# wnmusic/simpleFE

Measured on AMD Instinct MI355X. Metric: complex-float32 MS/s through 256-tap blkconv FIR; % of HBM roofline, higher is better.
Workload: dtype f32

## Files before the change

simplefe_amd/csrc/poly_gen.hip:

```cpp
#include <stdint.h>

#include <type_traits>

#ifdef SFE_DIAG
#include <stdlib.h>
#endif

#include "common.h"
#include "fft16.h"

namespace sfe {
namespace {

struct RunLds {
    double t0;
    float d;
    int k0;
    int count, pad;
};
static_assert(sizeof(RunLds) == 24, "TlSeg layout");

constexpr int GEN_MAX_RUNS = 1024;

template <int KPT, bool REAL, bool IN_U8, bool NOPRO = false>
__global__ __launch_bounds__(256, KPT <= 9 ? 3 : 2) void poly_gen4096_kernel(PolyGenArgs a)
{
    constexpr int NC = REAL ? 3 : 2;
    typedef typename std::conditional<REAL, float, v2f>::type E;
    __shared__ v2f lds[FFT_ROWS * LDS_K2_STRIDE];
    __shared__ unsigned tab_pos[KPT * 256];
    __shared__ float tab_mu[KPT * 256];
    __shared__ int s_bound[2 * NC], s_run[NC];
    const unsigned t = threadIdx.x, lo = t & 15u, hi = t >> 4;
    const int ch = blockIdx.y;
    const long long blk = (REAL ? 2 : 1) * (long long)blockIdx.x;
    const E *in = static_cast<const E *>(a.in) + (size_t)ch * a.in_stride;
    const E *hist = static_cast<const E *>(a.hist) + (size_t)ch * a.hl;
    E *out = static_cast<E *>(a.out) + (size_t)ch * a.out_stride;
    const int A = a.adv, U = a.U;

    v2f nx[16];
    const long long base = blk * A - a.ovl;
    if constexpr (IN_U8) {
        const unsigned char *in8 = static_cast<const unsigned char *>(a.in) + (size_t)ch * a.in_stride * (REAL ? 1 : 2);
        auto at = [&](long long i) -> E {
            if (i >= 0) {
                if (i >= a.n_in) return E{};
                if constexpr (REAL) return u8_to_f32(in8[i]);
                else return (v2f){u8_to_f32(in8[2 * i]), u8_to_f32(in8[2 * i + 1])};
            }
            return i >= -(long long)a.hl ? hist[a.hl + i] : E{};
        };
#pragma unroll
        for (int r = 0; r < 16; r++) {
            const long long i = base + 256 * r + (long long)t;
            if constexpr (REAL) nx[r] = (v2f){at(i), at(i + A)};
            else nx[r] = at(i);
        }
    } else if constexpr (!REAL) {
        if (base >= 0 && base + FFT_N <= a.n_in) {
#pragma unroll
            for (int r = 0; r < 16; r++) nx[r] = __builtin_nontemporal_load(in + base + 256 * r + t);
        } else {
#pragma unroll
            for (int r = 0; r < 16; r++) {
                const long long i = base + 256 * r + (long long)t;
                if (i >= 0) nx[r] = i < a.n_in ? in[i] : (v2f){0.0f, 0.0f};
                else nx[r] = i >= -(long long)a.hl ? hist[a.hl + i] : (v2f){0.0f, 0.0f};
            }
        }
    } else {
        if (base >= 0 && base + A + FFT_N <= a.n_in) {
#pragma unroll
            for (int r = 0; r < 16; r++)
                nx[r] = (v2f){__builtin_nontemporal_load(in + base + 256 * r + t), __builtin_nontemporal_load(in + base + A + 256 * r + t)};
        } else {
            auto at = [&](long long i) -> float {
                if (i >= 0) return i < a.n_in ? in[i] : 0.0f;
                return i >= -(long long)a.hl ? hist[a.hl + i] : 0.0f;
            };
#pragma unroll
            for (int r = 0; r < 16; r++) {
                const long long i = base + 256 * r + (long long)t;
                nx[r] = (v2f){at(i), at(i + A)};
            }
        }
    }

    int T = 0;
    long long k_first = 0;
    if constexpr (NOPRO) {
        T = a.diag_T < 256 * KPT ? a.diag_T : 256 * KPT;
        k_first = (long long)blockIdx.x * T;
        const unsigned Uu = (unsigned)U, e0 = (unsigned)a.ovl - 1u;
#pragma unroll
        for (int q = 0; q < KPT; q++) {
            const unsigned idx = t + 256u * q;
            const unsigned pl = (unsigned)(((unsigned long long)idx * (unsigned)A * Uu) / (unsigned)(T > 0 ? T : 1));
            const unsigned n = pl / Uu, ph = pl - n * Uu, e = e0 + (n < (unsigned)A ? n : (unsigned)A - 1u);
            const bool wrap = ph + 1u == Uu;
            const unsigned cell = (e >> 8) * LDS_K2_STRIDE + (e & 255u);
            const unsigned dcell = wrap ? ((e & 255u) == 255u ? LDS_K2_STRIDE - 255u : 1u) : 0u;
            tab_pos[idx] = (int)idx < T ? ((cell << 19) | (dcell << 10) | ((wrap ? 0u : ph + 1u) << 5) | ph) : (31u | (31u << 5));
            tab_mu[idx] = 0.25f;
        }
    } else {
    const long long Plo = (long long)U * (blk * A - 1), Phi = Plo + (long long)(REAL ? 2 : 1) * U * A;
    const long long BU = (long long)a.blksize * U;
    auto fdiv = [&](long long x) -> long long {
        if (x < 0) return 0;
        long long c = (long long)((double)x / (double)BU);
        if (c * BU > x) c--;
        if ((c + 1) * BU <= x) c++;
        return c;
    };
    long long c_first = fdiv(Plo + 1), c_last = fdiv(Phi);
    if (c_last >= a.n_chunks) c_last = a.n_chunks - 1;
    if (c_first > c_last) c_first = c_last;
    if (c_last > c_first + NC - 1) c_last = c_first + NC - 1;
    const int ncalls = (int)(c_last - c_first) + 1;
    SegChunk cc[NC];
    int nsg[NC], rbase[NC + 1];
    rbase[0] = 0;
#pragma unroll
    for (int i = 0; i < NC; i++) {
        cc[i] = a.chunks[c_first + (i < ncalls ? i : 0)];
        nsg[i] = i < ncalls ? cc[i].n_seg : 0;
        rbase[i + 1] = rbase[i] + nsg[i];
    }
    RunLds *runs = reinterpret_cast<RunLds *>(lds);
    {
        unsigned long long *ws = reinterpret_cast<unsigned long long *>(lds);
#pragma unroll
        for (int i = 0; i < NC; i++) {
            const unsigned long long *g = reinterpret_cast<const unsigned long long *>(static_cast<const RunLds *>(a.segs) + cc[i].seg_first);
            for (int j = (int)t; j < 3 * nsg[i]; j += 256) ws[3 * rbase[i] + j] = g[j];
        }
    }
    lds_barrier();
    auto count_below = [&](const RunLds *rs, int n_seg, int n_out, long long bound, int *run) -> int {
        *run = 0;
        if (n_seg == 0 || bound <= -1) return 0;
        const double bd = (double)bound;
        int l = 0, h = n_seg;
        while (l < h) {
            const int m = (l + h) >> 1;
            if (rs[m].t0 < bd) l = m + 1; else h = m;
        }
        if (l == 0) return 0;
        const RunLds g = rs[l - 1];
        long long i = g.count;
        if (g.count > 1 && g.d > 0.0f) {
            i = (long long)ceil((bd - g.t0) / (double)g.d);
            if (i < 0) i = 0;
            if (i > g.count) i = g.count;
            while (i < g.count && g.t0 + (double)i * (double)g.d < bd) i++;
            while (i > 0 && g.t0 + (double)(i - 1) * (double)g.d >= bd) i--;
        }
        *run = i < g.count ? l - 1 : l;
        const int k = g.k0 + (int)i;
        return k < n_out ? k : n_out;
    };
    const unsigned w = __builtin_amdgcn_readfirstlane(t >> 6), lane = t & 63u;
#pragma unroll
    for (int sx = 0; sx < 2 * NC; sx += 4) {
        const int sb = sx + (int)w;
        if (sb < 2 * NC) {
            int run = 0, r = 0;
#pragma unroll
            for (int i = 0; i < NC; i++)
                if (i == (sb >> 1) && i < ncalls)
                    r = count_below(runs + rbase[i], nsg[i], cc[i].n_out, ((sb & 1) ? Phi : Plo) - cc[i].in_off * U, &run);
            if (lane == 0) {
                s_bound[sb] = r;
                if (!(sb & 1)) s_run[sb >> 1] = run;
            }
        }
    }
    lds_barrier();
    int k_lo[NC], n_part[NC], idx_base[NC + 1], run_lo[NC];
    idx_base[0] = 0;
    k_first = cc[0].k_first + __builtin_amdgcn_readfirstlane(s_bound[0]);
    bool have_first = false;
#pragma unroll
    for (int i = 0; i < NC; i++) {
        k_lo[i] = __builtin_amdgcn_readfirstlane(s_bound[2 * i]);
        n_part[i] = __builtin_amdgcn_readfirstlane(s_bound[2 * i + 1]) - k_lo[i];
        run_lo[i] = __builtin_amdgcn_readfirstlane(s_run[i]);
        idx_base[i + 1] = idx_base[i] + n_part[i];
        if (!have_first && n_part[i] > 0) {
            k_first = cc[i].k_first + k_lo[i];
            have_first = true;
        }
    }
    T = idx_base[NC];
    if (T == 0) return;

#pragma unroll
    for (int q = 0; q < KPT; q++)
        if ((int)t + 256 * q >= T) {
            tab_pos[256 * q + t] = 31u | (31u << 5);
            tab_mu[256 * q + t] = 0.0f;
        }
    const unsigned Uu = (unsigned)U, Minv = Uu > 1u ? 0xFFFFFFFFu / Uu + 1u : 0u;
    const unsigned e0 = (unsigned)a.ovl - 1u;
#pragma unroll
    for (int part = 0; part < NC; part++) {
        const RunLds *rs = runs + rbase[part];
        const int ns = nsg[part];
        const unsigned off32 = (unsigned)(cc[part].in_off * U - Plo);
        int lu = run_lo[part];
        if (lu > ns - 1) lu = ns - 1;
#pragma unroll 1
        for (int c = (int)w; 64 * c < n_part[part]; c += 4) {
            const int kk0 = k_lo[part] + 64 * c;
            while (lu + 1 < ns && __builtin_amdgcn_readfirstlane(rs[lu].k0 + rs[lu].count) <= kk0) lu++;
            const int i_part = 64 * c + (int)lane;
            if (i_part < n_part[part]) {
                const int kk = kk0 + (int)lane;
                int l = lu;
                while (rs[l].k0 + rs[l].count <= kk) l++;
                const RunLds g = rs[l];
                const double tt = g.t0 + (double)(kk - g.k0) * (double)g.d;
                const double fl = floor(tt);
                const float mu = (float)(tt - fl);
                const unsigned pl = off32 + (unsigned)(int)fl;
                unsigned n = Uu > 1u ? __umulhi(pl, Minv) : pl;
                const unsigned ph = pl - n * Uu;
                unsigned half = 0u;
                if (REAL && n >= (unsigned)A) {
                    n -= (unsigned)A;
                    half = 1u;
                }
                const unsigned e = e0 + n;
                const bool wrap = ph + 1u == Uu;
                const unsigned cell = (e >> 8) * LDS_K2_STRIDE + (e & 255u);
                const unsigned dcell = wrap ? ((e & 255u) == 255u ? LDS_K2_STRIDE - 255u : 1u) : 0u;
                tab_pos[idx_base[part] + i_part] = (cell << 19) | (half << 15) | (dcell << 10) | ((wrap ? 0u : ph + 1u) << 5) | ph;
                tab_mu[idx_base[part] + i_part] = mu;
            }
        }
    }
    }
    lds_barrier();

    v2f p1[4], q1[4], p2[4], q2[4];
    auto load_tw1 = [&]() {
        unsigned tt = t;
        asm volatile("" : "+v"(tt));
#pragma unroll
        for (int k = 1; k < 4; k++) {
            p1[k] = a.tw1[k * 256 + tt];
            q1[k] = a.tw1[(k + 3) * 256 + tt];
        }
    };
    auto load_tw2 = [&]() {
        unsigned ll = lo;
        asm volatile("" : "+v"(ll));
#pragma unroll
        for (int k = 1; k < 4; k++) {
            p2[k] = a.tw2[k * 16 + ll];
            q2[k] = a.tw2[(k + 3) * 16 + ll];
        }
    };
    load_tw1();
    load_tw2();
    const unsigned base_b = hi * LDS_K2_STRIDE + lo, base_c = hi * LDS_K2_STRIDE + lo * LDS_K1_STRIDE;

    dft16<-1>(nx);
#pragma unroll
    for (int k = 0; k < 16; k++) {
        v2f x = nx[P16(k)];
        if ((k >> 2) && (k & 3)) x = cmul2(x, q1[k >> 2], p1[k & 3]);
        else if (k >> 2) x = cmul(x, q1[k >> 2]);
        else if (k & 3) x = cmul(x, p1[k & 3]);
        lds[t + (unsigned)k * LDS_K2_STRIDE] = x;
    }
    lds_barrier();
    v2f v[16];
#pragma unroll
    for (int r = 0; r < 16; r++) v[r] = lds[base_b + 16u * r];
    dft16<-1>(v);
    lds_barrier();
#pragma unroll
    for (int k = 0; k < 16; k++) {
        v2f x = v[P16(k)];
        if ((k >> 2) && (k & 3)) x = cmul2(x, q2[k >> 2], p2[k & 3]);
        else if (k >> 2) x = cmul(x, q2[k >> 2]);
        else if (k & 3) x = cmul(x, p2[k & 3]);
        lds[base_b + (unsigned)LDS_K1_STRIDE * k] = x;
    }
    lds_barrier();
    v2f hn[16];
    auto load_h = [&](int j) {
        unsigned tt = t;
        asm volatile("" : "+v"(tt));
        const v2f *hs = a.hs + (size_t)j * 16 * 256;
#pragma unroll
        for (int k = 0; k < 16; k++) hn[k] = hs[k * 256 + tt];
    };
    load_h(0);
    v2f X[16];
#pragma unroll
    for (int r = 0; r < 16; r++) X[r] = lds[base_c + r];
    dft16<-1>(X);

    E acc[KPT];
#pragma unroll
    for (int q = 0; q < KPT; q++) acc[q] = E{};
#pragma unroll 1
    for (int j = 0; j < U; j++) {
        lds_barrier();
#pragma unroll
        for (int k = 0; k < 16; k++) v[P16(k)] = cmul(X[P16(k)], hn[k]);
        if (j + 1 < U) load_h(j + 1);
        load_tw1();
        dft16_rev<+1>(v);
#pragma unroll
        for (int k = 0; k < 16; k++) lds[base_c + k] = v[k];
        lds_barrier();
#pragma unroll
        for (int r = 0; r < 16; r++) {
            v2f x = lds[base_b + (unsigned)LDS_K1_STRIDE * r];
            if ((r >> 2) && (r & 3)) x = cmul2_conj(x, q2[r >> 2], p2[r & 3]);
            else if (r >> 2) x = cmul_conj(x, q2[r >> 2]);
            else if (r & 3) x = cmul_conj(x, p2[r & 3]);
            v[r] = x;
        }
        dft16<+1>(v);
        lds_barrier();
#pragma unroll
        for (int k = 0; k < 16; k++) lds[base_b + 16u * k] = v[P16(k)];
        lds_barrier();
#pragma unroll
        for (int r = 0; r < 16; r++) {
            v2f x = lds[t + (unsigned)r * LDS_K2_STRIDE];
            if ((r >> 2) && (r & 3)) x = cmul2_conj(x, q1[r >> 2], p1[r & 3]);
            else if (r >> 2) x = cmul_conj(x, q1[r >> 2]);
            else if (r & 3) x = cmul_conj(x, p1[r & 3]);
            v[r] = x;
        }
        dft16<+1>(v);
#pragma unroll
        for (int r = 0; r < 16; r++) lds[t + (unsigned)r * LDS_K2_STRIDE] = v[P16(r)];
        lds_barrier();
        const unsigned ju = (unsigned)j;
        const char *lb = reinterpret_cast<const char *>(lds);
#pragma unroll
        for (int q = 0; q < KPT; q++) {
            const unsigned pw = tab_pos[256 * q + t];
            const float mu_q = tab_mu[256 * q + t];
            const float w0 = (pw & 31u) == ju ? 1.0f - mu_q : 0.0f;
            const float w1 = ((pw >> 5) & 31u) == ju ? mu_q : 0.0f;
            if constexpr (!REAL) {
                const unsigned a0 = pw >> 16;
                const v2f s0 = *reinterpret_cast<const v2f *>(lb + a0);
                const v2f s1 = *reinterpret_cast<const v2f *>(lb + a0 + (((pw >> 10) & 31u) << 3));
                acc[q] = __builtin_elementwise_fma((v2f){w0, w0}, s0, acc[q]);
                acc[q] = __builtin_elementwise_fma((v2f){w1, w1}, s1, acc[q]);
            } else {
                const unsigned a0 = (pw >> 16) + ((pw >> 13) & 4u);
                const float s0 = *reinterpret_cast<const float *>(lb + a0);
                const float s1 = *reinterpret_cast<const float *>(lb + a0 + (((pw >> 10) & 31u) << 3));
                acc[q] = __builtin_fmaf(w0, s0, acc[q]);
                acc[q] = __builtin_fmaf(w1, s1, acc[q]);
            }
        }
    }
#pragma unroll
    for (int q = 0; q < KPT; q++)
        if ((int)t + 256 * q < T) __builtin_nontemporal_store(acc[q], out + k_first + (long long)t + 256 * q);
}

}

int poly_gen_outputs_per_block(int U, int adv, float step)
{
    const double span = (double)U * adv;
    return (int)(span / ((double)step * (1.0 - 1.0 / 4194304.0))) + 2;
}

int launch_poly_gen(const PolyGenArgs &a0, int max_runs, float step, int n_channels, hipStream_t s)
{
    if (a0.n_chunks <= 0) return SFE_OK;
    PolyGenArgs a = a0;
    if (a.ovl < a.plen || a.ovl >= FFT_N / 2 || (a.ovl & 15) || max_runs > GEN_MAX_RUNS) return SFE_ESTATE;
    if (a.U > 31 || (long long)a.blksize * a.U >= 0x7fffffffLL) return SFE_ESTATE;
    const int per_wg = a.real ? 2 : 1, kpt_max = a.real ? 22 : 16;
    a.adv = FFT_N - a.ovl;
    if (poly_gen_outputs_per_block(a.U, per_wg * a.adv, step) > 256 * kpt_max) {
        a.adv = (int)((256.0 * kpt_max - 2) * (double)step * (1.0 - 1.0 / 4194304.0) / (a.U * per_wg)) & ~15;
        if (a.adv < 512 || poly_gen_outputs_per_block(a.U, per_wg * a.adv, step) > 256 * kpt_max) return SFE_ESTATE;
    }
    if (a.blksize < a.adv) return SFE_ESTATE;
    const int per_block = poly_gen_outputs_per_block(a.U, per_wg * a.adv, step);
    const long long A = a.adv;
    const long long nblk = (a.n_in / A + 1 + per_wg - 1) / per_wg;
    if (nblk > 0x7fffffffLL) return SFE_ESTATE;
    dim3 grid((unsigned)nblk, (unsigned)n_channels), block(256);
    const int kpt = (per_block + 255) / 256;
#ifdef SFE_DIAG
    if (const char *e = getenv("SFE_GEN_NOPRO"))
        if (atoi(e) && !a.real && !a.in_u8 && kpt <= 9) {
            a.diag_T = per_block - 3;
            hipLaunchKernelGGL((poly_gen4096_kernel<9, false, false, true>), grid, block, 0, s, a);
            SFE_HIP(hipGetLastError());
            return SFE_OK;
        }
#endif
#define SFE_GEN(KPTv, REALv)                                                                           \
    do {                                                                                              \
        if (a.in_u8) hipLaunchKernelGGL((poly_gen4096_kernel<KPTv, REALv, true>), grid, block, 0, s, a);      \
        else hipLaunchKernelGGL((poly_gen4096_kernel<KPTv, REALv, false>), grid, block, 0, s, a);            \
    } while (0)
    if (a.real) {
        if (kpt <= 12) SFE_GEN(12, true);
        else if (kpt <= 18) SFE_GEN(18, true);
        else SFE_GEN(22, true);
    } else {
        if (kpt <= 6) SFE_GEN(6, false);
        else if (kpt <= 9) SFE_GEN(9, false);
        else if (kpt <= 12) SFE_GEN(12, false);
        else SFE_GEN(16, false);
    }
#undef SFE_GEN
    SFE_HIP(hipGetLastError());
    return SFE_OK;
}

}
```

Measured before the change: 337,100.

## Replace double-precision run evaluation with fixed-point generator runs and ballot-based run search

Precomputes each segment run into a fixed-point GenRun (mantissa, step, shift), so per-output position and fractional offset come from integer arithmetic instead of double-precision multiply and floor. Bound search moves from a per-wave binary search with its extra barrier into the run-staging loop, and per-lane run lookup uses wave ballots instead of serial while loops. For U>1 the gather does one LDS load and FMA per output instead of two. This removes FP64 work and a barrier in the table-building prologue, at the cost of fixed-point precision assumptions and more complex setup code.

```diff
diff --git a/simplefe_amd/csrc/gentime.h b/simplefe_amd/csrc/gentime.h
--- /dev/null
+++ b/simplefe_amd/csrc/gentime.h
@@ -0,0 +1,82 @@
+#pragma once
+#include <math.h>
+#include <stdint.h>
+
+#if defined(__HIPCC__) || defined(__HIP__)
+#define SFE_GT_HD __host__ __device__
+#else
+#define SFE_GT_HD
+#endif
+
+namespace sfe {
+
+struct GenRun {
+    uint32_t m0;
+    uint32_t dsx;
+    int32_t  k0;
+    uint32_t pb;
+};
+
+struct GenLaw {
+    uint32_t m0, d;
+    int      s;
+};
+
+SFE_GT_HD inline bool gen_is_single(double t0, float d, int count) { return !(count > 1 && d > 0.0f && t0 >= 1.0); }
+
+SFE_GT_HD inline GenLaw gen_law(double t0, float d)
+{
+    int e;
+    (void)frexp(t0, &e);
+    const int s = e - 1 >= 23 ? 0 : 24 - e;
+    GenLaw g;
+    g.m0 = (uint32_t)ldexp(t0, s);
+    g.d = (uint32_t)ldexpf(d, s);
+    g.s = s;
+    return g;
+}
+
+SFE_GT_HD inline GenRun gen_run_make(double t0, float d, int k0, int count, uint32_t off)
+{
+    GenRun r;
+    r.k0 = k0;
+    if (gen_is_single(t0, d, count)) {
+        const double fl = floor(t0);
+        const float mu = (float)(t0 - fl);
+        union { float f; uint32_t u; } b;
+        b.f = mu;
+        r.m0 = b.u;
+        r.dsx = (31u << 24) | (1u << 31);
+        r.pb = off + (uint32_t)(int)fl;
+    } else {
+        const GenLaw g = gen_law(t0, d);
+        r.m0 = g.m0;
+        r.dsx = g.d | ((uint32_t)g.s << 24);
+        r.pb = off;
+    }
+    return r;
+}
+
+SFE_GT_HD inline void gen_run_at(const GenRun &r, int k, uint32_t *pos, float *mu)
+{
+    const uint32_t i = (uint32_t)(k - r.k0), s = (r.dsx >> 24) & 31u;
+    const uint32_t m = r.m0 + i * (r.dsx & 0xffffffu);
+    *pos = r.pb + (m >> s);
+    const float f = ldexpf((float)(m & ((1u << s) - 1u)), -(int)s);
+    union { uint32_t u; float f; } b;
+    b.u = r.m0;
+    *mu = (r.dsx >> 31) ? b.f : f;
+}
+
+SFE_GT_HD inline int gen_run_below(double t0, float d, int count, long long bound)
+{
+    if (!(t0 < (double)bound)) return 0;
+    if (gen_is_single(t0, d, count)) return count;
+    const GenLaw g = gen_law(t0, d);
+    if (bound > 0x80000000LL) bound = 0x80000000LL;
+    const long long x = (bound << g.s) - (long long)g.m0;
+    if (x > (long long)(count - 1) * g.d) return count;
+    return (int)(((uint32_t)x + g.d - 1u) / g.d);
+}
+
+}
diff --git a/simplefe_amd/csrc/poly_gen.hip b/simplefe_amd/csrc/poly_gen.hip
--- a/simplefe_amd/csrc/poly_gen.hip
+++ b/simplefe_amd/csrc/poly_gen.hip
@@ -8,6 +8,7 @@
 
 #include "common.h"
 #include "fft16.h"
+#include "gentime.h"
 
 namespace sfe {
 namespace {
@@ -121,63 +122,46 @@
     const int ncalls = (int)(c_last - c_first) + 1;
     SegChunk cc[NC];
     int nsg[NC], rbase[NC + 1];
+    unsigned off32[NC];
     rbase[0] = 0;
 #pragma unroll
     for (int i = 0; i < NC; i++) {
         cc[i] = a.chunks[c_first + (i < ncalls ? i : 0)];
         nsg[i] = i < ncalls ? cc[i].n_seg : 0;
         rbase[i + 1] = rbase[i] + nsg[i];
-    }
-    RunLds *runs = reinterpret_cast<RunLds *>(lds);
-    {
-        unsigned long long *ws = reinterpret_cast<unsigned long long *>(lds);
-#pragma unroll
-        for (int i = 0; i < NC; i++) {
-            const unsigned long long *g = reinterpret_cast<const unsigned long long *>(static_cast<const RunLds *>(a.segs) + cc[i].seg_first);
-            for (int j = (int)t; j < 3 * nsg[i]; j += 256) ws[3 * rbase[i] + j] = g[j];
+        off32[i] = (unsigned)(cc[i].in_off * U - Plo);
+    }
+    GenRun *runs = reinterpret_cast<GenRun *>(lds);
+    const RunLds *gsegs = static_cast<const RunLds *>(a.segs);
+#pragma unroll
+    for (int i = 0; i < NC; i++) {
+        const long long lo = Plo - cc[i].in_off * U, hi = Phi - cc[i].in_off * U;
+        if (nsg[i] == 0) {
+            if (t == 0) {
+                s_bound[2 * i] = s_bound[2 * i + 1] = 0;
+                s_run[i] = 0;
+            }
+            continue;
+        }
+        for (int j = (int)t; j < nsg[i]; j += 256) {
+            const RunLds g = gsegs[cc[i].seg_first + j];
+            const double tn = j + 1 < nsg[i] ? gsegs[cc[i].seg_first + j + 1].t0 : __builtin_inf();
+            runs[rbase[i] + j] = gen_run_make(g.t0, g.d, g.k0, g.count, off32[i]);
+#pragma unroll
+            for (int h = 0; h < 2; h++) {
+                const long long bd = h ? hi : lo;
+                const bool in_run = g.t0 < (double)bd && !(tn < (double)bd);
+                if (in_run || (j == 0 && !(g.t0 < (double)bd))) {
+                    const int below = in_run ? gen_run_below(g.t0, g.d, g.count, bd) : 0;
+                    const int k = in_run ? g.k0 + below : 0;
+                    s_bound[2 * i + h] = k < cc[i].n_out ? k : cc[i].n_out;
+                    if (!h) s_run[i] = in_run && below >= g.count ? j + 1 : j;
+                }
+            }
         }
     }
     lds_barrier();
-    auto count_below = [&](const RunLds *rs, int n_seg, int n_out, long long bound, int *run) -> int {
-        *run = 0;
-        if (n_seg == 0 || bound <= -1) return 0;
-        const double bd = (double)bound;
-        int l = 0, h = n_seg;
-        while (l < h) {
-            const int m = (l + h) >> 1;
-            if (rs[m].t0 < bd) l = m + 1; else h = m;
-        }
-        if (l == 0) return 0;
-        const RunLds g = rs[l - 1];
-        long long i = g.count;
-        if (g.count > 1 && g.d > 0.0f) {
-            i = (long long)ceil((bd - g.t0) / (double)g.d);
-            if (i < 0) i = 0;
-            if (i > g.count) i = g.count;
-            while (i < g.count && g.t0 + (double)i * (double)g.d < bd) i++;
-            while (i > 0 && g.t0 + (double)(i - 1) * (double)g.d >= bd) i--;
-        }
-        *run = i < g.count ? l - 1 : l;
-        const int k = g.k0 + (int)i;
-        return k < n_out ? k : n_out;
-    };
     const unsigned w = __builtin_amdgcn_readfirstlane(t >> 6), lane = t & 63u;
-#pragma unroll
-    for (int sx = 0; sx < 2 * NC; sx += 4) {
-        const int sb = sx + (int)w;
-        if (sb < 2 * NC) {
-            int run = 0, r = 0;
-#pragma unroll
-            for (int i = 0; i < NC; i++)
-                if (i == (sb >> 1) && i < ncalls)
-                    r = count_below(runs + rbase[i], nsg[i], cc[i].n_out, ((sb & 1) ? Phi : Plo) - cc[i].in_off * U, &run);
-            if (lane == 0) {
-                s_bound[sb] = r;
-                if (!(sb & 1)) s_run[sb >> 1] = run;
-            }
-        }
-    }
-    lds_barrier();
     int k_lo[NC], n_part[NC], idx_base[NC + 1], run_lo[NC];
     idx_base[0] = 0;
     k_first = cc[0].k_first + __builtin_amdgcn_readfirstlane(s_bound[0]);
@@ -196,8 +180,8 @@
     T = idx_base[NC];
     if (T == 0) return;
 
-#pragma unroll
-    for (int q = 0; q < KPT; q++)
+#pragma unroll 1
+    for (int q = T >> 8; q < KPT; q++)
         if ((int)t + 256 * q >= T) {
             tab_pos[256 * q + t] = 31u | (31u << 5);
             tab_mu[256 * q + t] = 0.0f;
@@ -206,27 +190,31 @@
     const unsigned e0 = (unsigned)a.ovl - 1u;
 #pragma unroll
     for (int part = 0; part < NC; part++) {
-        const RunLds *rs = runs + rbase[part];
+        const GenRun *rs = runs + rbase[part];
         const int ns = nsg[part];
-        const unsigned off32 = (unsigned)(cc[part].in_off * U - Plo);
         int lu = run_lo[part];
         if (lu > ns - 1) lu = ns - 1;
 #pragma unroll 1
         for (int c = (int)w; 64 * c < n_part[part]; c += 4) {
-            const int kk0 = k_lo[part] + 64 * c;
-            while (lu + 1 < ns && __builtin_amdgcn_readfirstlane(rs[lu].k0 + rs[lu].count) <= kk0) lu++;
+            const int kk0 = k_lo[part] + 64 * c, kk = kk0 + (int)lane;
+            int l = lu;
+            for (int r0 = lu + 1;; r0 += 64) {
+                const int r = r0 + (int)lane;
+                const int kr = rs[r < ns ? r : ns - 1].k0;
+                const int kn = r < ns ? kr : 0x7fffffff;
+                const int nb = __popcll(__ballot(kn <= kk0)), nin = __popcll(__ballot(kn <= kk0 + 63));
+                l += nb;
+                for (int x = nb; x < nin; x++) l += kk >= __builtin_amdgcn_readlane(kn, x) ? 1 : 0;
+                lu += nb;
+                if (nin < 64) break;
+            }
             const int i_part = 64 * c + (int)lane;
             if (i_part < n_part[part]) {
-                const int kk = kk0 + (int)lane;
-                int l = lu;
-                while (rs[l].k0 + rs[l].count <= kk) l++;
-                const RunLds g = rs[l];
-                const double tt = g.t0 + (double)(kk - g.k0) * (double)g.d;
-                const double fl = floor(tt);
-                const float mu = (float)(tt - fl);
-                const unsigned pl = off32 + (unsigned)(int)fl;
+                unsigned pl;
+                float mu;
+                gen_run_at(rs[l], kk, &pl, &mu);
                 unsigned n = Uu > 1u ? __umulhi(pl, Minv) : pl;
-                const unsigned ph = pl - n * Uu;
+                const unsigned ph = pl - __umul24(n, Uu);
                 unsigned half = 0u;
                 if (REAL && n >= (unsigned)A) {
                     n -= (unsigned)A;
@@ -346,24 +334,43 @@
         lds_barrier();
         const unsigned ju = (unsigned)j;
         const char *lb = reinterpret_cast<const char *>(lds);
-#pragma unroll
-        for (int q = 0; q < KPT; q++) {
-            const unsigned pw = tab_pos[256 * q + t];
-            const float mu_q = tab_mu[256 * q + t];
-            const float w0 = (pw & 31u) == ju ? 1.0f - mu_q : 0.0f;
-            const float w1 = ((pw >> 5) & 31u) == ju ? mu_q : 0.0f;
-            if constexpr (!REAL) {
-                const unsigned a0 = pw >> 16;
-                const v2f s0 = *reinterpret_cast<const v2f *>(lb + a0);
-                const v2f s1 = *reinterpret_cast<const v2f *>(lb + a0 + (((pw >> 10) & 31u) << 3));
-                acc[q] = __builtin_elementwise_fma((v2f){w0, w0}, s0, acc[q]);
-                acc[q] = __builtin_elementwise_fma((v2f){w1, w1}, s1, acc[q]);
-            } else {
-                const unsigned a0 = (pw >> 16) + ((pw >> 13) & 4u);
-                const float s0 = *reinterpret_cast<const float *>(lb + a0);
-                const float s1 = *reinterpret_cast<const float *>(lb + a0 + (((pw >> 10) & 31u) << 3));
-                acc[q] = __builtin_fmaf(w0, s0, acc[q]);
-                acc[q] = __builtin_fmaf(w1, s1, acc[q]);
+        if (U == 1) {
+#pragma unroll
+            for (int q = 0; q < KPT; q++) {
+                const unsigned pw = tab_pos[256 * q + t];
+                const float mu_q = tab_mu[256 * q + t];
+                const float w0 = (pw & 31u) == ju ? 1.0f - mu_q : 0.0f;
+                const float w1 = ((pw >> 5) & 31u) == ju ? mu_q : 0.0f;
+                if constexpr (!REAL) {
+                    const unsigned a0 = pw >> 16;
+                    const v2f s0 = *reinterpret_cast<const v2f *>(lb + a0);
+                    const v2f s1 = *reinterpret_cast<const v2f *>(lb + a0 + (((pw >> 10) & 31u) << 3));
+                    acc[q] = __builtin_elementwise_fma((v2f){w0, w0}, s0, acc[q]);
+                    acc[q] = __builtin_elementwise_fma((v2f){w1, w1}, s1, acc[q]);
+                } else {
+                    const unsigned a0 = (pw >> 16) + ((pw >> 13) & 4u);
+                    const float s0 = *reinterpret_cast<const float *>(lb + a0);
+                    const float s1 = *reinterpret_cast<const float *>(lb + a0 + (((pw >> 10) & 31u) << 3));
+                    acc[q] = __builtin_fmaf(w0, s0, acc[q]);
+                    acc[q] = __builtin_fmaf(w1, s1, acc[q]);
+                }
+            }
+        } else {
+#pragma unroll
+            for (int q = 0; q < KPT; q++) {
+                const unsigned pw = tab_pos[256 * q + t];
+                const float mu_q = tab_mu[256 * q + t];
+                const bool second = ((pw >> 5) & 31u) == ju;
+                const float wt = (pw & 31u) == ju ? 1.0f - mu_q : (second ? mu_q : 0.0f);
+                unsigned a0 = (pw >> 16) + (second ? ((pw >> 10) & 31u) << 3 : 0u);
+                if constexpr (!REAL) {
+                    const v2f sj = *reinterpret_cast<const v2f *>(lb + a0);
+                    acc[q] = __builtin_elementwise_fma((v2f){wt, wt}, sj, acc[q]);
+                } else {
+                    a0 += (pw >> 13) & 4u;
+                    const float sj = *reinterpret_cast<const float *>(lb + a0);
+                    acc[q] = __builtin_fmaf(wt, sj, acc[q]);
+                }
             }
         }
     }
```

Result: no change. 335,300 (median of 3 runs) (-0.5%).
